# biodatageeks/polars-bio

Measured on AMD Instinct MI355X. Metric: overlap-pairs/sec, higher is better.
Workload: dtype int32; 1 GPU; overlap_100M_5M_24contig; probe_rows=100000000, build_rows=5000000, contigs=24, filter_op=Strict, parallelism=single GPU

## Files before the change

### polars-bio_amd/csrc/cslice.hip.h

```cpp
#pragma once
#include "slice.hip.h"

namespace ivj {

constexpr int CS_THREADS = 1024;
constexpr int CS_WAVES = CS_THREADS / kWave;
constexpr int CS_ITEMS = 4;
constexpr int CS_TILE = CS_THREADS * CS_ITEMS;
constexpr int CS_WTILE = kWave * CS_ITEMS;
constexpr int CS_MAX_CONTIGS = 256;
constexpr int CS_WIN = 12;
constexpr int CS_LIN = 4;
constexpr int CS_POS_BIAS = 1 << 23;
static_assert((long long)SL_MAX_BUCKETS * SL_MAX_ROWS <= CS_POS_BIAS, "an index of this path must fit a staging entry's row field");
constexpr int CS_BIN_STRIDE_PAD = 2;

constexpr int CS_CUR_STRIDE = 1;
constexpr int CS_META_FMT = 8;
constexpr unsigned long long CS_STATE_REC8 = 8ull;
constexpr int CS_REC8_GIVE_UP = 3;
__host__ __device__ __forceinline__ int cs_bits_for(uint32_t v) { int b = 0; while (b < 32 && (v >> b) != 0) ++b; return b == 0 ? 1 : b; }

typedef int cs_rec __attribute__((ext_vector_type(3), aligned(4)));
typedef int cs_rec8 __attribute__((ext_vector_type(2), aligned(8)));
// ... 687 lines not shown
    __syncthreads();
    uint32_t mlen = 0, moff = 0;
    const int64_t n_groups = (n + (int64_t)CS_SGROUP * CS_SRATE - 1) / ((int64_t)CS_SGROUP * CS_SRATE);
    for (int64_t t = (int64_t)bid * CS_THREADS + threadIdx.x; t < n_groups * CS_SGROUP; t += (int64_t)nblocks * CS_THREADS) {
        const int64_t i = (t / CS_SGROUP) * ((int64_t)CS_SGROUP * CS_SRATE) + (t % CS_SGROUP);
        if (i < n) {
            const int32_t qe = pe[i], qs = ps[i];
            const uint32_t b = cs_bucket<STRICT>(l_spl, l_cm, l_cell, g.nb, g.n_contigs, pc[i], qe);
            atomicAdd(&h[b], 1u);
            if (b < (uint32_t)g.nb) {
                const uint32_t len = qe >= qs ? (uint32_t)qe - (uint32_t)qs : 0x7fffffffu;
                const uint32_t off = (uint32_t)qe - (uint32_t)unflip((uint32_t)l_spl[b]);
                mlen = len > mlen ? len : mlen;
                moff = off > moff ? off : moff;
            }
        }
    }
#pragma unroll
    for (int d = kWave / 2; d > 0; d >>= 1) {
        const uint32_t a = __shfl_xor(mlen, d, kWave), b = __shfl_xor(moff, d, kWave);
        mlen = a > mlen ? a : mlen; moff = b > moff ? b : moff;
    }
    if ((threadIdx.x & (kWave - 1)) == 0) { atomicMax(&h[g.nb + 1], mlen); atomicMax(&h[g.nb + 2], moff); }
    __syncthreads();
    for (int k = threadIdx.x; k <= g.nb; k += CS_THREADS) if (h[k]) atomicAdd(&gh[k], h[k]);
    if (threadIdx.x == 0) { atomicMax(&gh[g.nb + 1], h[g.nb + 1]); atomicMax(&gh[g.nb + 2], h[g.nb + 2]); }
}
template <bool STRICT>
__global__ __launch_bounds__(CS_THREADS) void k_cs_sample_hist(CsTab tab, CsGeom g, const int32_t* __restrict__ pc, const int32_t* __restrict__ ps,
                                                              const int32_t* __restrict__ pe, int64_t n, uint32_t* __restrict__ gh) {
    extern __shared__ __attribute__((aligned(16))) unsigned char cs_lds[];
    cs_sample_body<STRICT>(cs_lds, blockIdx.x, gridDim.x, tab, g, pc, ps, pe, n, gh);
}
template <bool STRICT>
__global__ __launch_bounds__(CS_THREADS) void k_cs_bins_sample(int n_bins, const int32_t* __restrict__ bound, const int32_t* __restrict__ b_start,
                                                              const int2* __restrict__ ep, const int32_t* __restrict__ b_contig,
                                                              const int32_t* __restrict__ seg, int R, unsigned short* __restrict__ bins,
                                                              int4* __restrict__ smeta, int32_t* __restrict__ far_rows,
                                                              CsTab tab, CsGeom g, const int32_t* __restrict__ pc, const int32_t* __restrict__ ps,
                                                              const int32_t* __restrict__ pe, int64_t n, uint32_t* __restrict__ gh) {
    extern __shared__ __attribute__((aligned(16))) unsigned char cs_lds[];
    __shared__ uint32_t wmin[CS_WAVES];
    if ((int)blockIdx.x < n_bins) cs_bins_body(cs_lds, wmin, (int)blockIdx.x, bound, b_start, ep, b_contig, seg, R, bins, smeta, far_rows);
    else cs_sample_body<STRICT>(cs_lds, blockIdx.x - (unsigned)n_bins, gridDim.x - (unsigned)n_bins, tab, g, pc, ps, pe, n, gh);
}

__global__ __launch_bounds__(CS_THREADS) void k_cs_regions(const uint32_t* __restrict__ gh, int nb, uint32_t slack, int allow8, uint32_t* __restrict__ rstart,
                                                          uint32_t* __restrict__ rcur, int32_t* __restrict__ meta, const int32_t* __restrict__ far_src,
                                                          uint32_t* __restrict__ hw, uint32_t hw_seq) {
    if (threadIdx.x == 0 && hw) {
        hw_store(hw + 4, (uint32_t)__hip_atomic_load(far_src, __ATOMIC_RELAXED, __HIP_MEMORY_SCOPE_AGENT));
        hw_store(hw + 5, hw_seq);
    }
    if (threadIdx.x == 0) {
        int lb = 0;
        if (allow8) {
            const unsigned long long ml = (unsigned long long)gh[nb + 1] * 2ull + 64ull;
            const unsigned long long mo = (unsigned long long)gh[nb + 2] + gh[nb + 2] / 4 + 4096ull;
            const int lbits = ml > 0xffffffffull ? 33 : cs_bits_for((uint32_t)ml);
            const int obits = mo > 0xffffffffull ? 33 : cs_bits_for((uint32_t)mo);
            if (lbits + obits <= 32) lb = 32 - obits;
        }
        meta[CS_META_FMT] = lb;
    }
    __shared__ __attribute__((aligned(16))) int wsum[CS_WAVES];
    constexpr int OWN = (SL_MAX_BUCKETS + 1 + CS_THREADS - 1) / CS_THREADS;
    uint32_t cap[OWN];
    long long mine = 0;
#pragma unroll
    for (int q = 0; q < OWN; ++q) {
        const int b = OWN * threadIdx.x + q;
        cap[q] = 0;
        if (b < nb) {
            const unsigned long long est = (unsigned long long)gh[b] * CS_SRATE;
            unsigned long long c = est + est / 4 + slack;
            c = (c + 31ull) & ~31ull;
            cap[q] = (uint32_t)c;
        }
        mine += cap[q];
    }
    long long total;
    long long pre = sl_block_exclusive_sum_i32<CS_WAVES>((int)mine, wsum, &total);
#pragma unroll
    for (int q = 0; q < OWN; ++q) {
        const int b = OWN * threadIdx.x + q;
        if (b < nb) { rstart[b] = (uint32_t)pre; rcur[(size_t)b * CS_CUR_STRIDE] = 0u; }
// ... 1463 lines not shown
```

### polars-bio_amd/csrc/host_core.hip.h

```cpp
#pragma once

namespace {

thread_local std::string g_err;

int fail(int code, const std::string& msg) { g_err = msg; return code; }

#define HIP_TRY(expr)                                                                         \
    do {                                                                                      \
        hipError_t _e = (expr);                                                               \
        if (_e != hipSuccess)                                                                 \
            return fail(IVJ_EHIP, std::string(#expr) + ": " + hipGetErrorString(_e));         \
    } while (0)

#define IVJ_ABI_CATCH                                                                                     \
    catch (const std::bad_alloc&) { return fail(IVJ_ENOMEM, "host allocation failed (std::bad_alloc)"); }   \
    catch (const std::exception& e) { return fail(IVJ_ESTATE, std::string("internal error: ") + e.what()); } \
    catch (...) { return fail(IVJ_ESTATE, "internal error: unknown exception"); }

#define IVJ_TRY(expr)                 \
    do {                              \
        int _r = (expr);              \
        if (_r != IVJ_OK) return _r;  \
    } while (0)
// ... 31 lines not shown
        for (int k = 0; k < 2; ++k) {
            if (buf[k]) (void)hipHostFree(buf[k]);
            if (ev[k]) (void)hipEventDestroy(ev[k]);
            buf[k] = nullptr; ev[k] = nullptr;
        }
    }
};

inline std::atomic<int> g_live_contexts{0};

struct ivj_ctx {
    ivj_ctx() { g_live_contexts.fetch_add(1, std::memory_order_relaxed); }
    ~ivj_ctx() { g_live_contexts.fetch_sub(1, std::memory_order_relaxed); }
    ivj_ctx(const ivj_ctx&) = delete;
    ivj_ctx& operator=(const ivj_ctx&) = delete;
    int device = 0;
    hipStream_t own_stream = nullptr;
    hipStream_t stream = nullptr;
    Arena arena;
    char* ov_buf = nullptr;
    size_t ov_cap = 0;
    int64_t ov_n = -1;
    const void* ov_probe_start = nullptr;
    const void *ov_probe_contig = nullptr, *ov_probe_end = nullptr;
    const ivj_index* ov_ix = nullptr;
    int32_t ov_filter = -1;
    int32_t* ov_hi = nullptr;
    int32_t* ov_cnt = nullptr;
    long long* ov_tile = nullptr;
    long long* h_total = nullptr;
    uint32_t* hw = nullptr;
    uint32_t* hw_dev = nullptr;
    uint32_t hw_seq = 0;
    uint32_t cs_far_hw_seq = 0;
    uint32_t cs_fused_hw_seq = 0;
    int env_spin_us = 4000;
    long long hw_misses = 0;
    bool cs_prep_zero = false;
    XferSlots xfer;
    char* nl_cache = nullptr;
    size_t nl_cache_cap = 0;
    int env_nearest_lines = -1;
    char* ix_cache = nullptr;
    size_t ix_cache_cap = 0;
    int64_t ov_total = 0;
    bool ov_part = false;
    int32_t *pt_c = nullptr, *pt_s = nullptr, *pt_e = nullptr, *pt_row = nullptr;
    uint32_t* pt_off = nullptr; int pt_ntiles = 0;
    uint32_t* pt_bstart = nullptr;
    bool part_attr_set = false;
    bool os_attr_set = false;
    hipEvent_t cs_event = nullptr;
    const ivj_index* cs_far_owner = nullptr;
    hipEvent_t ix3_event = nullptr;
    bool ix3_attr_set = false;
    int env_ix_merge = -1;
    int env_ix_stage = -1;
    int env_ix_v3 = -1;
    int ix3_fallback_streak = 0;
    unsigned ix3_builds_since_fallback = 0;
    int64_t ix3_fallbacks = 0;
    struct StreamBufs { int32_t* h_in = nullptr; int32_t* d_in = nullptr; size_t in_cap = 0; char* d_out = nullptr; size_t d_out_cap = 0;
                        char* h_out = nullptr; size_t h_out_cap = 0; } st_cache[3];
    char* lb_buf = nullptr; size_t lb_cap = 0;
    char* sl_buf = nullptr;
    size_t sl_cap = 0;
    int4* sl_rec = nullptr;
    uint2* sl_cache = nullptr;
    uint32_t *sl_gh = nullptr, *sl_rstart = nullptr, *sl_rcur = nullptr, *sl_bend = nullptr;
    bool sl_sampled = false;
    uint32_t *sl_blk = nullptr, *sl_part = nullptr, *sl_bstart = nullptr;
    int32_t* sl_meta = nullptr;
    int2* sl_map = nullptr;
    long long *sl_tile = nullptr, *sl_tpart = nullptr;
    bool ov_slice = false;
    bool ov_cs = false;
    bool sl_plan_valid = false;
    int sl_items = 2;
    int env_joint_bins = 0, env_count_nolds = 0, env_count_ablate = 0;
    int sl_env_rows = 0, sl_env_chunk = 0, sl_env_notab = 0, sl_env_nobins = 0, sl_env_ablate = 0, sl_env_auto = 1, sl_env_stable = 0, sl_env_sthreads = 1024;
    SlicePlan sl_plan;
    bool cs_sattr_set = false;
    bool cs_attr_set = false;
    int cs_env_walk = -1;
    int cs_env_off = 0;
    int cs_env_ptile = 0;
    int cs_env_fill_two = 0;
    int cs_env_sampled = 1;
    int cs_env_slack = 0;
    int64_t cs_sampled_overflows = 0;
    bool cs_force_exact = false;
    int cs_env_fuse_sample = 1;
    int cs_env_rec8 = 1;
    bool cs_force_rec12 = false;
    int cs_rec8_streak = 0;
    unsigned cs_rec8_skipped = 0;
    bool cs_rec8_tried = false;
    int64_t cs_rec8_overflows = 0;
    int cs_env_nocache = 0;
    int cs_env_persist = 1;
    int cs_env_pmax = 0, cs_env_pgrain = 0;
    int cs_env_pchunks = 0;
    int n_cus = 0;
    const char* cs_env_wgtrace = nullptr;
    unsigned long long* cs_trace_buf = nullptr;
    size_t cs_trace_cap = 0;
    int timing = 0;
    bool t_open = false;
    std::vector<TimingRec> recs;
    std::vector<hipEvent_t> pool;
    size_t pool_used = 0;
    std::vector<ivj_index*> live;
    std::vector<struct ivj_stream*> streams;
    std::vector<struct ivj_comm*> comms;
};

inline void spin_relax(int i, bool crowded) {
#if !defined(__HIP_DEVICE_COMPILE__) && (defined(__x86_64__) || defined(__i386__))
    __builtin_ia32_pause();
#endif
    if (crowded && (i & 7) == 7) std::this_thread::yield();
}
template <typename Query>
inline bool spin_wait(ivj_ctx* ctx, Query&& q, hipError_t* out) {
    if (ctx->env_spin_us <= 0) return false;
// ... 36 lines not shown
    int32_t* seg = nullptr;
    int32_t* flags = nullptr;
    int32_t* e_end = nullptr;
    int32_t* e_pos = nullptr;
    int4* cmeta = nullptr;
    uint32_t* bins = nullptr;
    int4* cmeta_e = nullptr;
    uint32_t* bins_e = nullptr;
    int4* brec = nullptr;
    int4* brec_e = nullptr;
    int32_t* pargmax = nullptr;
    char* ix3_z = nullptr;
    int4* nrec = nullptr;
    int4* cmeta_j = nullptr;
    int4* crec = nullptr;
    int64_t bins_len = 0;
    bool has_end_order = false, has_end_table = false;
    bool has_argmax = false;
    int4* nline = nullptr;
    size_t nline_cap = 0;
    bool has_lines = false;
    unsigned long long* psum = nullptr;
    size_t psum_stride = 0;
    bool has_psum = false;
    bool has_flat = false;
    bool has_rec4 = false;
    unsigned long long* spl = nullptr;
    int sl_R = 0, sl_nb = 0, sl_ncells = -1;
    int4* sl_cm = nullptr;
    uint32_t* sl_cell = nullptr;
    CsGeom cs_g{0, 0, 0, 0, 0};
    bool cs_ok = false, cs_built = false;
    bool cs_far_pending = false;
    bool cs_walk = false;
    int64_t cs_far = 0;
    int32_t* cs_bound = nullptr;
    unsigned long long* cs_spl = nullptr;
    int4* cs_cm = nullptr;
    uint32_t* cs_cell = nullptr;
    unsigned short* cs_bins = nullptr;
    int4* cs_smeta = nullptr;
    int32_t* hier = nullptr;
    bool hier_built = false;
    bool tables_built = false;
    bool has_tables = true;
    char* slab = nullptr;
    size_t slab_cap = 0;
};

namespace {

struct DeviceGuard {
    int prev = -1;
    bool ok = true;
    explicit DeviceGuard(int dev) {
        if (hipGetDevice(&prev) != hipSuccess) prev = -1;
        if (prev != dev) ok = hipSetDevice(dev) == hipSuccess;
    }
    ~DeviceGuard() { if (prev >= 0) (void)hipSetDevice(prev); }
};

int arena_reserve(ivj_ctx* ctx, size_t bytes) {
    Arena& A = ctx->arena;
    A.off = 0;
    if (bytes <= A.cap) return IVJ_OK;
    HIP_TRY(hipStreamSynchronize(ctx->stream));
// ... 166 lines not shown
```

### polars-bio_amd/csrc/host_cslice.hip.h

```cpp
#pragma once

namespace {

constexpr int CS_MIN_ROWS = 3072;
bool cs_geom(int64_t n, int nc, int want_rows, CsGeom& g) {
    if (n <= 0 || nc < 1 || nc > CS_MAX_CONTIGS) return false;
    const int64_t extra = (nc < n ? nc : n) + 1;
    int64_t min_rows = CS_MIN_ROWS;
    if (const char* ev = std::getenv("IVJ_CS_MIN_ROWS")) { const int v = std::atoi(ev); if (v > 0) min_rows = v; }
    int64_t R = want_rows > 0 ? want_rows : std::max<int64_t>((n + 1023) / 1024, min_rows);
    R = (R + 63) / 64 * 64;
    if (n / R + extra > SL_MAX_BUCKETS) {
        if (extra + 8 >= SL_MAX_BUCKETS) return false;
        R = ((n + (SL_MAX_BUCKETS - extra) - 1) / (SL_MAX_BUCKETS - extra) + 63) / 64 * 64;
    }
    if (R > SL_MAX_ROWS) return false;
    g.R = (int)R;
    g.nb = (int)(n / R + extra);
    g.n_contigs = nc;
    g.cps = 0; g.ncells = 0;
    for (int cps = 4; cps >= 1 && !g.ncells; cps >>= 1) {
        const int cells = cps * g.nb + 2 * nc;
        if ((size_t)cs_part_lds(g.nb, cells, nc, 4).total <= 160 * 1024) { g.ncells = cells; g.cps = cps; }
    }
    return g.ncells != 0;
}

size_t cs_index_bytes(const CsGeom& g) {
    return align_up((size_t)(g.nb + 2) * 4) + align_up((size_t)g.nb * 8) + align_up((size_t)CS_MAX_CONTIGS * 16) + align_up((size_t)g.ncells * 4) +
           align_up((size_t)g.nb * (size_t)(2 * g.R + CS_BIN_STRIDE_PAD) * 2) + align_up((size_t)g.nb * 32);
}
void cs_index_carve(ivj_index* ix, char* p) {
    const CsGeom& g = ix->cs_g;
    ix->cs_bound = (int32_t*)p; p += align_up((size_t)(g.nb + 2) * 4);
    ix->cs_spl = (unsigned long long*)p; p += align_up((size_t)g.nb * 8);
    ix->cs_cm = (int4*)p; p += align_up((size_t)CS_MAX_CONTIGS * 16);
    ix->cs_cell = (uint32_t*)p; p += align_up((size_t)g.ncells * 4);
    ix->cs_bins = (unsigned short*)p; p += align_up((size_t)g.nb * (size_t)(2 * g.R + CS_BIN_STRIDE_PAD) * 2);
    ix->cs_smeta = (int4*)p;
}

bool cs_wanted(const ivj_ctx* ctx, const ivj_index* ix, const ivj_opts* opts) {
    if (!ix->cs_ok || ctx->cs_env_off) return false;
    if (opts->slice_rows > 0 && ((opts->slice_rows + 63) / 64 * 64) != ix->cs_g.R) return false;
    return true;
}

constexpr double CS_FAR_LIMIT = 5e-4;

struct CsSampleArgs { bool strict; const int32_t *pc, *ps, *pe; int64_t n; uint32_t* gh; unsigned sgrid; size_t lds; };

int cs_ensure_tables(ivj_ctx* ctx, ivj_index* ix, const CsSampleArgs* sample = nullptr) {
    if (ix->cs_built) return IVJ_OK;
    const CsGeom& g = ix->cs_g;
    const bool pz = ctx->cs_prep_zero && sample != nullptr;
    LAUNCH(ctx, "cs_prep", k_cs_prep, 1, CS_THREADS, (const int32_t*)ix->seg, (const int32_t*)ix->b_start, g, ix->cs_bound, ix->cs_spl, ix->cs_cm, ix->cs_cell,
           pz ? reinterpret_cast<uint32_t*>(ctx->sl_meta + 4) : (uint32_t*)nullptr, pz ? 16 : 0, pz ? ctx->sl_gh : (uint32_t*)nullptr, pz ? g.nb + 4 : 0);
    const size_t lds = (size_t)4 * g.R + (size_t)2 * (2 * g.R + 8);
    if (sample) {
        const CsTab tab{ix->cs_spl, ix->cs_cm, ix->cs_cell};
        const size_t l2 = std::max(lds, sample->lds);
        with_bool(sample->strict, [&](auto S) {
            LAUNCH_LDS(ctx, "cs_bins_sample", (k_cs_bins_sample<S>), (unsigned)g.nb + sample->sgrid, CS_THREADS, l2, g.nb, (const int32_t*)ix->cs_bound, (const int32_t*)ix->b_start,
                       (const int2*)ix->ep, (const int32_t*)ix->b_contig, (const int32_t*)ix->seg, g.R, ix->cs_bins, ix->cs_smeta, ix->flags + 1, tab, g, sample->pc, sample->ps,
                       sample->pe, sample->n, sample->gh);
        });
    } else {
        LAUNCH_LDS(ctx, "cs_bins", k_cs_bins, g.nb, CS_THREADS, lds, (const int32_t*)ix->cs_bound, (const int32_t*)ix->b_start, (const int2*)ix->ep,
                   (const int32_t*)ix->b_contig, (const int32_t*)ix->seg, g.R, ix->cs_bins, ix->cs_smeta, ix->flags + 1);
    }
    HIP_TRY(hipGetLastError());
    if (!ctx->cs_event) HIP_TRY(hipEventCreateWithFlags(&ctx->cs_event, hipEventDisableTiming));
    if (sample && ctx->hw) ctx->cs_far_hw_seq = ++ctx->hw_seq;
    else {
        ctx->cs_far_hw_seq = 0;
        HIP_TRY(hipMemcpyAsync(ctx->h_total + 5, ix->flags + 1, 4, hipMemcpyDeviceToHost, ctx->stream));
        HIP_TRY(hipEventRecord(ctx->cs_event, ctx->stream));
    }
    ix->cs_far_pending = true;
    ctx->cs_far_owner = ix;
    ix->cs_built = true;
    return IVJ_OK;
}

int cs_resolve_tables(ivj_ctx* ctx, ivj_index* ix) {
    if (!ix->cs_far_pending) return IVJ_OK;
    bool have = false;
    if (ctx->cs_far_owner == ix) {
        HIP_TRY(wait_event(ctx, ctx->cs_event));
        ctx->cs_far_owner = nullptr;
        if (ctx->cs_far_hw_seq == 0) { ix->cs_far = *reinterpret_cast<const int32_t*>(ctx->h_total + 5); have = true; }
        else if (reinterpret_cast<volatile uint32_t*>(ctx->hw)[5] == ctx->cs_far_hw_seq) { ix->cs_far = (int32_t)reinterpret_cast<volatile uint32_t*>(ctx->hw)[4]; have = true; }
        else ++ctx->hw_misses;
    }
    if (!have) {
        HIP_TRY(hipMemcpyAsync(ctx->h_total + 5, ix->flags + 1, 4, hipMemcpyDeviceToHost, ctx->stream));
        HIP_TRY(hipStreamSynchronize(ctx->stream));
        ix->cs_far = *reinterpret_cast<const int32_t*>(ctx->h_total + 5);
    }
    const double share = ix->n > 0 ? (double)ix->cs_far / (double)ix->n : 0.0;
    ix->cs_walk = ctx->cs_env_walk >= 0 ? ctx->cs_env_walk != 0 : share > CS_FAR_LIMIT;
    ix->cs_far_pending = false;
    if (ix->cs_walk) IVJ_TRY(ensure_hier(ctx, ix));
    return IVJ_OK;
}

bool cs_sampled_wanted(const ivj_ctx* ctx, int64_t n, bool stable) {
    return !stable && ctx->cs_env_sampled != 0 && !ctx->cs_force_exact && n >= (1ll << 16) && n <= (1ll << 30);
}
uint32_t cs_region_slack(const ivj_ctx* ctx, const CsGeom& g, int64_t n) {
    if (ctx->cs_env_slack > 0) return (uint32_t)((ctx->cs_env_slack + 31) & ~31);
    return (uint32_t)((4 * CS_TILE + n / (16 * (int64_t)(g.nb > 0 ? g.nb : 1)) + 31) & ~31ll);
}
int64_t cs_record_capacity(const ivj_ctx* ctx, const CsGeom& g, int64_t n) {
    return n + n / 4 + n / 32 + (int64_t)(cs_region_slack(ctx, g, n) + 64) * (g.nb + 2) + 4 * CS_TILE;
}

int cs_plan(const ivj_ctx* ctx, const ivj_index* ix, int64_t n, const ivj_opts* opts, SlicePlan& P, int& wcap) {
    const CsGeom& g = ix->cs_g;
    P.g.nb = g.nb; P.g.R = g.R; P.g.ncells = g.ncells; P.g.cps = g.cps;
    int64_t chunk = ((n + 2047) / 2048 + 2 * CS_TILE - 1) / (2 * CS_TILE) * (2 * CS_TILE);
    if (chunk < 2 * CS_TILE) chunk = 2 * CS_TILE;
    if (chunk > 16 * CS_TILE) chunk = 16 * CS_TILE;
    P.chunk = (int)chunk;
    P.nchunks = (int)((n + chunk - 1) / chunk);
    P.items = CS_ITEMS;
    const int want_chunk = opts->slice_chunk > 0 ? opts->slice_chunk : ctx->sl_env_chunk;
    int64_t jchunk = want_chunk > 0 ? ((int64_t)want_chunk + CS_TILE - 1) / CS_TILE * CS_TILE
                                    : (n >= (32ll << 20) ? 4 * CS_TILE : (n >= (8ll << 20) ? 2 * CS_TILE : CS_TILE));
    if (want_chunk <= 0 && n >= (32ll << 20)) {
        const int64_t a = n / (g.nb > 0 ? g.nb : 1);
// ... 28 lines not shown
}

int cs_partition(ivj_ctx* ctx, ivj_index* ix, const ivj_side* probe, const ivj_opts* opts, const SlicePlan& P, bool stable) {
    const int64_t n = probe->n;
    const CsGeom& g = ix->cs_g;
    const bool strict = opts->filter_op == IVJ_FILTER_STRICT;
    ctx->sl_sampled = cs_sampled_wanted(ctx, n, stable);
    const bool fuse_sample = ctx->sl_sampled && !ix->cs_built && ctx->cs_env_fuse_sample != 0;
    if (!fuse_sample) IVJ_TRY(cs_ensure_tables(ctx, ix));
    const CsTab tab{ix->cs_spl, ix->cs_cm, ix->cs_cell};
    const bool vec = aligned16(probe->contig) && aligned16(probe->start) && aligned16(probe->end) && (!probe->row_id || aligned16(probe->row_id));
    const size_t hist_lds = (size_t)16 * CS_MAX_CONTIGS + (size_t)8 * g.nb + (size_t)4 * g.ncells + 4 * (g.nb + 1);
    const size_t hist = (size_t)(g.nb + 1) * (size_t)P.nchunks;
    if (!ctx->cs_attr_set) {
        IVJ_TRY(set_dyn_lds(&k_cs_hist<true>, 96 * 1024)); IVJ_TRY(set_dyn_lds(&k_cs_hist<false>, 96 * 1024));
        IVJ_TRY(set_dyn_lds((&k_cs_scatter<true, 4, false>), 160 * 1024)); IVJ_TRY(set_dyn_lds((&k_cs_scatter<false, 4, false>), 160 * 1024));
        IVJ_TRY(set_dyn_lds((&k_cs_scatter<true, 8, false>), 160 * 1024));
        IVJ_TRY(set_dyn_lds(&k_cs_join<true, CS_FUSED>, 160 * 1024)); IVJ_TRY(set_dyn_lds(&k_cs_join<false, CS_FUSED>, 160 * 1024));
        IVJ_TRY(set_dyn_lds(&k_cs_join<true, CS_COUNT>, 160 * 1024)); IVJ_TRY(set_dyn_lds(&k_cs_join<false, CS_COUNT>, 160 * 1024));
        IVJ_TRY(set_dyn_lds(&k_cs_join<true, CS_FILL>, 160 * 1024)); IVJ_TRY(set_dyn_lds(&k_cs_join<false, CS_FILL>, 160 * 1024));
        IVJ_TRY(set_dyn_lds(&k_cs_join_plain<true, CS_FUSED>, 160 * 1024)); IVJ_TRY(set_dyn_lds(&k_cs_join_plain<false, CS_FUSED>, 160 * 1024));
        IVJ_TRY(set_dyn_lds(&k_cs_join_plain<true, CS_COUNT>, 160 * 1024)); IVJ_TRY(set_dyn_lds(&k_cs_join_plain<false, CS_COUNT>, 160 * 1024));
        IVJ_TRY(set_dyn_lds(&k_cs_join_plain<true, CS_FILL>, 160 * 1024)); IVJ_TRY(set_dyn_lds(&k_cs_join_plain<false, CS_FILL>, 160 * 1024));
        IVJ_TRY(set_dyn_lds(&k_cs_scatter_stable<true>, 160 * 1024)); IVJ_TRY(set_dyn_lds(&k_cs_scatter_stable<false>, 160 * 1024));
        IVJ_TRY(set_dyn_lds(&k_cs_fill<true, false, false>, 160 * 1024)); IVJ_TRY(set_dyn_lds(&k_cs_fill<false, false, false>, 160 * 1024));
        IVJ_TRY(set_dyn_lds(&k_cs_fill<true, false, true>, 160 * 1024)); IVJ_TRY(set_dyn_lds(&k_cs_fill<false, false, true>, 160 * 1024));
        IVJ_TRY(set_dyn_lds(&k_cs_fill<true, true, false>, 160 * 1024)); IVJ_TRY(set_dyn_lds(&k_cs_fill<false, true, false>, 160 * 1024));
        ctx->cs_attr_set = true;
    }
    int32_t* rec = reinterpret_cast<int32_t*>(ctx->sl_rec);
    if (ctx->sl_sampled) {
        if (!ctx->cs_sattr_set) {
            IVJ_TRY(set_dyn_lds(&k_cs_sample_hist<true>, 96 * 1024)); IVJ_TRY(set_dyn_lds(&k_cs_sample_hist<false>, 96 * 1024));
            IVJ_TRY(set_dyn_lds(&k_cs_bins_sample<true>, 96 * 1024)); IVJ_TRY(set_dyn_lds(&k_cs_bins_sample<false>, 96 * 1024));
            IVJ_TRY(set_dyn_lds((&k_cs_scatter<true, 4, true>), 160 * 1024)); IVJ_TRY(set_dyn_lds((&k_cs_scatter<false, 4, true>), 160 * 1024));
            IVJ_TRY(set_dyn_lds((&k_cs_scatter<true, 8, true>), 160 * 1024)); IVJ_TRY(set_dyn_lds((&k_cs_scatter<false, 8, true>), 160 * 1024));
            IVJ_TRY(set_dyn_lds((&k_cs_scatter<true, 4, true, true>), 160 * 1024)); IVJ_TRY(set_dyn_lds((&k_cs_scatter<false, 4, true, true>), 160 * 1024));
            IVJ_TRY(set_dyn_lds((&k_cs_scatter<true, 8, true, true>), 160 * 1024)); IVJ_TRY(set_dyn_lds((&k_cs_scatter<false, 8, true, true>), 160 * 1024));
            IVJ_TRY(set_dyn_lds((&k_cs_scatter12k<true, 12>), 160 * 1024)); IVJ_TRY(set_dyn_lds((&k_cs_scatter12k<false, 12>), 160 * 1024));
            IVJ_TRY(set_dyn_lds((&k_cs_scatter12k<true, 16>), 160 * 1024)); IVJ_TRY(set_dyn_lds((&k_cs_scatter12k<false, 16>), 160 * 1024));
            ctx->cs_sattr_set = true;
        }
        const bool pz = ctx->cs_prep_zero && fuse_sample;
        if (!pz) HIP_TRY(hipMemsetAsync(ctx->sl_gh, 0, (size_t)(g.nb + 4) * 4, ctx->stream));
        const int64_t n_samp = (n + CS_SRATE - 1) / CS_SRATE;
        const unsigned sgrid = (unsigned)std::min<int64_t>(256, (n_samp + CS_THREADS - 1) / CS_THREADS);
        if (fuse_sample) {
            const CsSampleArgs sa{strict, probe->contig, probe->start, probe->end, n, ctx->sl_gh, sgrid, hist_lds + 16};
            IVJ_TRY(cs_ensure_tables(ctx, ix, &sa));
        } else {
            with_bool(strict, [&](auto S) {
                LAUNCH_LDS(ctx, "cs_sample", (k_cs_sample_hist<S>), sgrid, CS_THREADS, hist_lds + 16, tab, g, probe->contig, probe->start, probe->end, n, ctx->sl_gh);
            });
        }
        const bool sticky12 = ctx->cs_rec8_streak >= CS_REC8_GIVE_UP && (++ctx->cs_rec8_skipped & 63) != 0;
        const int allow8 = (ctx->cs_env_rec8 != 0 && !ctx->cs_force_rec12 && !sticky12) ? 1 : 0;
        ctx->cs_rec8_tried = allow8 != 0;
        const bool far_hw = fuse_sample && ix->cs_far_pending && ctx->cs_far_owner == ix && ctx->cs_far_hw_seq != 0;
        LAUNCH(ctx, "cs_regions", k_cs_regions, 1, CS_THREADS, (const uint32_t*)ctx->sl_gh, g.nb, cs_region_slack(ctx, g, n), allow8, ctx->sl_rstart, ctx->sl_rcur, ctx->sl_meta,
               (const int32_t*)(ix->flags + 1), far_hw ? ctx->hw_dev : (uint32_t*)nullptr, ctx->cs_far_hw_seq);
        if (far_hw) HIP_TRY(hipEventRecord(ctx->cs_event, ctx->stream));
        unsigned long long* state = reinterpret_cast<unsigned long long*>(ctx->sl_meta + 4);
        if (allow8) t_begin(ctx, "cs_scatter");
        auto scatter = [&](auto R8) {
            with_bool(strict, P.part_items == 8, [&](auto S, auto I8) {
                hipLaunchKernelGGL((k_cs_scatter<S, I8 ? 8 : 4, true, R8>), dim3(P.nchunks), dim3(CS_THREADS), P.part_lds, ctx->stream, tab, g, probe->contig, probe->start,
                                   probe->end, probe->row_id, n, P.chunk, P.nchunks, vec, (const uint32_t*)ctx->sl_rstart, ctx->sl_rcur, state, (const int32_t*)ctx->sl_meta, rec, ctx->sl_env_ablate);
            });
        };
        if (allow8) {
            if (P.part12) {
                const int wide = (P.part16 && !probe->row_id) ? 16 : 12;
                const size_t ldsw = (size_t)cs_part12_lds(g.nb, g.ncells, g.n_contigs, wide).total;
                unsigned long long* ptrace = nullptr;
                const char* ptrace_path = std::getenv("IVJ_CS_PTRACE");
                if (ptrace_path && ptrace_path[0]) {
                    HIP_TRY(hipMalloc((void**)&ptrace, (size_t)P.nchunks * 64));
                    HIP_TRY(hipMemsetAsync(ptrace, 0, (size_t)P.nchunks * 64, ctx->stream));
                }
                with_bool(strict, wide == 16, [&](auto S, auto W16) {
                    hipLaunchKernelGGL((k_cs_scatter12k<S, W16 ? 16 : 12>), dim3(P.nchunks), dim3(CS_THREADS), ldsw, ctx->stream, tab, g, probe->contig, probe->start, probe->end, probe->row_id, n,
                                       P.chunk, P.nchunks, vec, (const uint32_t*)ctx->sl_rstart, ctx->sl_rcur, state, (const int32_t*)ctx->sl_meta, rec, ctx->sl_env_ablate, ptrace);
                });
                if (ptrace) {
                    std::vector<unsigned long long> h((size_t)P.nchunks * 8);
                    HIP_TRY(hipStreamSynchronize(ctx->stream));
                    HIP_TRY(hipMemcpy(h.data(), ptrace, h.size() * 8, hipMemcpyDeviceToHost));
                    (void)hipFree(ptrace);
                    if (FILE* f = std::fopen(ptrace_path, "ab")) {
                        const unsigned long long head[4] = {0x50545243ull, (unsigned long long)P.nchunks, (unsigned long long)P.chunk, (unsigned long long)wide};
                        std::fwrite(head, 8, 4, f); std::fwrite(h.data(), 8, h.size(), f); std::fclose(f);
                    }
                }
            }
// ... 211 lines not shown
```

### polars-bio_amd/csrc/ivjoin.hip

```cpp
#include "../../include/ivjoin.h"

#include <hip/hip_runtime.h>

#include <algorithm>
#include <atomic>
#include <chrono>
#include <cstdio>
#include <cstdlib>
#include <cstring>
#include <string>
#include <vector>
#include <thread>
#include <type_traits>

#include "probe.hip.h"
#include "slice.hip.h"
#include "cslice.hip.h"
#include "onesweep.hip.h"
#include "ixsort3.hip.h"
#include "scan.hip.h"
#include "group.hip.h"
#include "depth.hip.h"
#include "depth_sum.hip.h"
#include "depth_query.hip.h"
// ... 40 lines not shown
int ivj_ctx_create(int device, ivj_ctx** out) try {
    if (!out) return fail(IVJ_EINVAL, "out is NULL");
    int cnt = 0;
    IVJ_TRY(ivj_device_count(&cnt));
    if (device < 0 || device >= cnt) return fail(IVJ_EHIP, "no usable HIP device " + std::to_string(device) + " (device count " + std::to_string(cnt) + ")");
    HIP_TRY(hipSetDevice(device));
    ivj_ctx* ctx = new ivj_ctx();
    ctx->device = device;
    { int cus = 0; if (hipDeviceGetAttribute(&cus, hipDeviceAttributeMultiprocessorCount, device) == hipSuccess) ctx->n_cus = cus; }
    hipError_t e = hipStreamCreateWithFlags(&ctx->own_stream, hipStreamNonBlocking);
    if (e != hipSuccess) { delete ctx; return fail(IVJ_EHIP, std::string("hipStreamCreate: ") + hipGetErrorString(e)); }
    ctx->stream = ctx->own_stream;
    if (const char* ev = std::getenv("IVJ_SLICE_ITEMS")) ctx->sl_items = std::atoi(ev) == 4 ? 4 : 2;
    if (const char* ev = std::getenv("IVJ_SLICE_ROWS")) ctx->sl_env_rows = std::atoi(ev);
    if (const char* ev = std::getenv("IVJ_SLICE_CHUNK")) ctx->sl_env_chunk = std::atoi(ev);
    if (const char* ev = std::getenv("IVJ_SLICE_NOTAB")) ctx->sl_env_notab = std::atoi(ev);
    if (const char* ev = std::getenv("IVJ_SLICE_NOBINS")) ctx->sl_env_nobins = std::atoi(ev);
    if (const char* ev = std::getenv("IVJ_SLICE_ABLATE")) ctx->sl_env_ablate = std::atoi(ev);
    if (const char* ev = std::getenv("IVJ_SLICE_AUTO")) ctx->sl_env_auto = std::atoi(ev);
    if (const char* ev = std::getenv("IVJ_SLICE_STABLE")) ctx->sl_env_stable = std::atoi(ev);
    if (const char* ev = std::getenv("IVJ_SLICE_SCATTER_THREADS")) ctx->sl_env_sthreads = std::atoi(ev);
    if (const char* ev = std::getenv("IVJ_CS")) ctx->cs_env_off = std::atoi(ev) == 0 ? 1 : 0;
    if (const char* ev = std::getenv("IVJ_CS_PTILE")) ctx->cs_env_ptile = std::atoi(ev);
    if (const char* ev = std::getenv("IVJ_CS_NOCACHE")) ctx->cs_env_nocache = std::atoi(ev);
    if (const char* ev = std::getenv("IVJ_CS_PERSIST")) ctx->cs_env_persist = std::atoi(ev);
    if (const char* ev = std::getenv("IVJ_CS_PCHUNKS")) ctx->cs_env_pchunks = std::atoi(ev);
    if (const char* ev = std::getenv("IVJ_CS_PMAX")) ctx->cs_env_pmax = std::atoi(ev);
    if (const char* ev = std::getenv("IVJ_CS_PGRAIN")) ctx->cs_env_pgrain = std::atoi(ev);
    if (const char* ev = std::getenv("IVJ_CS_WGTRACE")) ctx->cs_env_wgtrace = ev[0] ? ev : nullptr;
    if (const char* ev = std::getenv("IVJ_CS_SAMPLED")) ctx->cs_env_sampled = std::atoi(ev);
    if (const char* ev = std::getenv("IVJ_CS_SLACK")) ctx->cs_env_slack = std::atoi(ev);
    if (const char* ev = std::getenv("IVJ_CS_REC8")) ctx->cs_env_rec8 = std::atoi(ev);
    if (const char* ev = std::getenv("IVJ_CS_FUSE_SAMPLE")) ctx->cs_env_fuse_sample = std::atoi(ev);
    if (const char* ev = std::getenv("IVJ_CS_FILL_TWO")) ctx->cs_env_fill_two = std::atoi(ev);
    if (const char* ev = std::getenv("IVJ_CS_WALK")) ctx->cs_env_walk = std::atoi(ev) != 0 ? 1 : 0;
    if (const char* ev = std::getenv("IVJ_JOINT_BINS")) ctx->env_joint_bins = std::atoi(ev);
    if (const char* ev = std::getenv("IVJ_COUNT_ABLATE")) ctx->env_count_ablate = std::atoi(ev);
    if (const char* ev = std::getenv("IVJ_NEAREST_LINES")) ctx->env_nearest_lines = std::atoi(ev);
    if (const char* ev = std::getenv("IVJ_COUNT_NOLDS")) ctx->env_count_nolds = std::atoi(ev);
    if (const char* ev = std::getenv("IVJ_IX_V3")) ctx->env_ix_v3 = std::atoi(ev) != 0 ? 1 : 0;
    if (const char* ev = std::getenv("IVJ_SPIN_US")) ctx->env_spin_us = std::atoi(ev);
    if (const char* ev = std::getenv("IVJ_IX_MERGE")) ctx->env_ix_merge = std::atoi(ev);
    if (const char* ev = std::getenv("IVJ_IX_STAGE")) ctx->env_ix_stage = std::atoi(ev) != 0 ? 1 : 0;
    e = hipHostMalloc((void**)&ctx->h_total, 64, hipHostMallocDefault);
    if (e != hipSuccess) { (void)hipStreamDestroy(ctx->own_stream); delete ctx; return fail(IVJ_EHIP, std::string("hipHostMalloc: ") + hipGetErrorString(e)); }
    {
        const char* ev = std::getenv("IVJ_HOST_WORDS");
        if (!(ev && std::atoi(ev) == 0)) {
            void* hp = nullptr;
            void* dp = nullptr;
            if (hipHostMalloc(&hp, 256, hipHostMallocMapped | hipHostMallocCoherent) == hipSuccess) {
                if (hipHostGetDevicePointer(&dp, hp, 0) == hipSuccess && dp) {
                    std::memset(hp, 0, 256);
                    ctx->hw = (uint32_t*)hp; ctx->hw_dev = (uint32_t*)dp;
                } else (void)hipHostFree(hp);
            }
            (void)hipGetLastError();
        }
    }
    *out = ctx;
    return IVJ_OK;
} IVJ_ABI_CATCH

namespace {
void stream_release(ivj_stream* st, bool keep_cache);
void free_stream_bufs(ivj_ctx::StreamBufs& b) {
    if (b.h_in) (void)hipHostFree(b.h_in);
    if (b.d_in) (void)hipFree(b.d_in);
    if (b.d_out) (void)hipFree(b.d_out);
    if (b.h_out) (void)hipHostFree(b.h_out);
    b = ivj_ctx::StreamBufs();
}
}

void ivj_ctx_destroy(ivj_ctx* ctx) {
    if (!ctx) return;
    DeviceGuard g(ctx->device);
    (void)hipStreamSynchronize(ctx->stream);
    while (!ctx->streams.empty()) stream_release(ctx->streams.back(), false);
    for (ivj_index* ix : ctx->live) ix->ctx = nullptr;
    for (ivj_comm* cm : ctx->comms) comm_detach(cm);
    if (ctx->arena.base) (void)hipFree(ctx->arena.base);
    if (ctx->ov_buf) (void)hipFree(ctx->ov_buf);
    if (ctx->sl_buf) (void)hipFree(ctx->sl_buf);
    if (ctx->cs_trace_buf) (void)hipFree(ctx->cs_trace_buf);
    if (ctx->lb_buf) (void)hipFree(ctx->lb_buf);
    for (auto& cb : ctx->st_cache) free_stream_bufs(cb);
    if (ctx->ix_cache) (void)hipFree(ctx->ix_cache);
    if (ctx->nl_cache) (void)hipFree(ctx->nl_cache);
    if (ctx->ix3_event) (void)hipEventDestroy(ctx->ix3_event);
    if (ctx->cs_event) (void)hipEventDestroy(ctx->cs_event);
    if (ctx->h_total) (void)hipHostFree(ctx->h_total);
    if (std::getenv("IVJ_DEBUG_REDO")) std::fprintf(stderr, "[ivj] context: host words %s, %lld misses of %u; ix3 fallbacks %lld\n", ctx->hw ? "on" : "off", (long long)ctx->hw_misses, ctx->hw_seq, (long long)ctx->ix3_fallbacks);
    if (ctx->hw) (void)hipHostFree(ctx->hw);
    ctx->xfer.release();
    for (hipEvent_t ev : ctx->pool) (void)hipEventDestroy(ev);
    if (ctx->own_stream) (void)hipStreamDestroy(ctx->own_stream);
    delete ctx;
}

int ivj_ctx_set_stream(ivj_ctx* ctx, void* hip_stream) try {
    if (!ctx) return fail(IVJ_EINVAL, "ctx is NULL");
    HIP_TRY(hipStreamSynchronize(ctx->stream));
    ctx->stream = (hip_stream == (void*)-1) ? ctx->own_stream : (hipStream_t)hip_stream;
    return IVJ_OK;
} IVJ_ABI_CATCH

int ivj_ctx_sync(ivj_ctx* ctx) try {
    if (!ctx) return fail(IVJ_EINVAL, "ctx is NULL");
    HIP_TRY(hipStreamSynchronize(ctx->stream));
    return IVJ_OK;
} IVJ_ABI_CATCH

namespace ivj { __global__ void k_profile_mark() {} }

int ivj_ctx_profile_mark(ivj_ctx* ctx) try {
    if (!ctx) return fail(IVJ_EINVAL, "ctx is NULL");
    DeviceGuard g(ctx->device);
    hipLaunchKernelGGL(ivj::k_profile_mark, dim3(1), dim3(1), 0, ctx->stream);
    HIP_TRY(hipGetLastError());
    return IVJ_OK;
} IVJ_ABI_CATCH

int ivj_ctx_enable_timing(ivj_ctx* ctx, int on) try {
// ... 10 lines not shown
    HIP_TRY(hipStreamSynchronize(ctx->stream));
    std::vector<ivj_timing> agg;
    for (const TimingRec& r : ctx->recs) {
        float ms = 0.f;
        if (hipEventElapsedTime(&ms, r.a, r.b) != hipSuccess) continue;
        size_t j = 0;
        for (; j < agg.size(); ++j) if (std::strcmp(agg[j].name, r.name) == 0) break;
        if (j == agg.size()) {
            ivj_timing t; std::memset(&t, 0, sizeof t);
            std::strncpy(t.name, r.name, sizeof(t.name) - 1);
            agg.push_back(t);
        }
        agg[j].launches += 1; agg[j].ms += ms;
    }
    *n = (int)agg.size();
    for (int i = 0; i < (int)agg.size() && i < cap; ++i) out[i] = agg[i];
    ctx->recs.clear();
    ctx->pool_used = 0;
    return IVJ_OK;
} IVJ_ABI_CATCH


int ivj_index_build_dev(ivj_ctx* ctx, const ivj_side* build_dev, const ivj_opts* opts, int with_end_order, ivj_index** out) try {
    if (!ctx || !out) return fail(IVJ_EINVAL, "ctx or out is NULL");
    IVJ_TRY(check_opts(opts));
    IVJ_TRY(check_side(build_dev, "build"));
    DeviceGuard g(ctx->device);
    return index_build(ctx, build_dev, opts, with_end_order, out);
} IVJ_ABI_CATCH

void ivj_index_free(ivj_index* ix) {
    if (!ix) return;
    ivj_ctx* ctx = ix->ctx;
    if (ctx) {
        if (ctx->ov_ix == ix) { ctx->ov_ix = nullptr; ctx->ov_n = -1; }
        for (size_t k = 0; k < ctx->live.size(); ++k)
            if (ctx->live[k] == ix) { ctx->live[k] = ctx->live.back(); ctx->live.pop_back(); break; }
    }
    if (ix->nline) {
        if (ctx && ix->nline_cap > ctx->nl_cache_cap) {
            char* old = ctx->nl_cache;
            ctx->nl_cache = reinterpret_cast<char*>(ix->nline); ctx->nl_cache_cap = ix->nline_cap;
            if (old) { DeviceGuard g(ctx->device); (void)hipFree(old); }
        } else {
            DeviceGuard g(ix->device);
            (void)hipFree(ix->nline);
        }
    }
    if (ix->psum) {
        DeviceGuard g(ix->device);
        (void)hipFree(ix->psum);
    }
    if (ix->slab) {
        if (ctx && ix->slab_cap > ctx->ix_cache_cap) {
            char* old = ctx->ix_cache;
            ctx->ix_cache = ix->slab; ctx->ix_cache_cap = ix->slab_cap;
            if (old) { DeviceGuard g(ctx->device); (void)hipFree(old); }
        } else {
            DeviceGuard g(ix->device);
            (void)hipFree(ix->slab);
        }
    }
    delete ix;
}

int ivj_overlap_count_dev(ivj_ctx* ctx, ivj_index* ix, const ivj_side* probe_dev, const ivj_opts* opts, int64_t* n_pairs) try {
// ... 1127 lines not shown
```

Measured before the change: 111.4 billion overlap-pairs/s.

## Run cs_bins on a side stream concurrently with probe sampling instead of fusing kernels

Replaces the fused bins+sample kernel with separate kernels. On first build, the bin-table kernel runs on a forked non-blocking side stream while the sampling histogram runs on the main stream. The main stream joins via an event when tables are resolved. The far-count readback moves to a pinned memcpy plus event, dropping the host-word path in the regions kernel. This adds stream, event and lifetime handling, and the benefit only applies when tables are not already built.

Result: no change. 111.8 billion overlap-pairs/s, median of 3 (+0.4%).

```diff
diff --git a/polars-bio_amd/csrc/cslice.hip.h b/polars-bio_amd/csrc/cslice.hip.h
--- a/polars-bio_amd/csrc/cslice.hip.h
+++ b/polars-bio_amd/csrc/cslice.hip.h
@@ -743,26 +743,9 @@
     extern __shared__ __attribute__((aligned(16))) unsigned char cs_lds[];
     cs_sample_body<STRICT>(cs_lds, blockIdx.x, gridDim.x, tab, g, pc, ps, pe, n, gh);
 }
-template <bool STRICT>
-__global__ __launch_bounds__(CS_THREADS) void k_cs_bins_sample(int n_bins, const int32_t* __restrict__ bound, const int32_t* __restrict__ b_start,
-                                                              const int2* __restrict__ ep, const int32_t* __restrict__ b_contig,
-                                                              const int32_t* __restrict__ seg, int R, unsigned short* __restrict__ bins,
-                                                              int4* __restrict__ smeta, int32_t* __restrict__ far_rows,
-                                                              CsTab tab, CsGeom g, const int32_t* __restrict__ pc, const int32_t* __restrict__ ps,
-                                                              const int32_t* __restrict__ pe, int64_t n, uint32_t* __restrict__ gh) {
-    extern __shared__ __attribute__((aligned(16))) unsigned char cs_lds[];
-    __shared__ uint32_t wmin[CS_WAVES];
-    if ((int)blockIdx.x < n_bins) cs_bins_body(cs_lds, wmin, (int)blockIdx.x, bound, b_start, ep, b_contig, seg, R, bins, smeta, far_rows);
-    else cs_sample_body<STRICT>(cs_lds, blockIdx.x - (unsigned)n_bins, gridDim.x - (unsigned)n_bins, tab, g, pc, ps, pe, n, gh);
-}
 
 __global__ __launch_bounds__(CS_THREADS) void k_cs_regions(const uint32_t* __restrict__ gh, int nb, uint32_t slack, int allow8, uint32_t* __restrict__ rstart,
-                                                          uint32_t* __restrict__ rcur, int32_t* __restrict__ meta, const int32_t* __restrict__ far_src,
-                                                          uint32_t* __restrict__ hw, uint32_t hw_seq) {
-    if (threadIdx.x == 0 && hw) {
-        hw_store(hw + 4, (uint32_t)__hip_atomic_load(far_src, __ATOMIC_RELAXED, __HIP_MEMORY_SCOPE_AGENT));
-        hw_store(hw + 5, hw_seq);
-    }
+                                                          uint32_t* __restrict__ rcur, int32_t* __restrict__ meta) {
     if (threadIdx.x == 0) {
         int lb = 0;
         if (allow8) {
diff --git a/polars-bio_amd/csrc/host_core.hip.h b/polars-bio_amd/csrc/host_core.hip.h
--- a/polars-bio_amd/csrc/host_core.hip.h
+++ b/polars-bio_amd/csrc/host_core.hip.h
@@ -87,7 +87,6 @@
     uint32_t* hw = nullptr;
     uint32_t* hw_dev = nullptr;
     uint32_t hw_seq = 0;
-    uint32_t cs_far_hw_seq = 0;
     uint32_t cs_fused_hw_seq = 0;
     int env_spin_us = 4000;
     long long hw_misses = 0;
@@ -107,6 +106,8 @@
     bool os_attr_set = false;
     hipEvent_t cs_event = nullptr;
     const ivj_index* cs_far_owner = nullptr;
+    hipStream_t cs_side = nullptr;
+    hipEvent_t cs_fork = nullptr;
     hipEvent_t ix3_event = nullptr;
     bool ix3_attr_set = false;
     int env_ix_merge = -1;
@@ -146,6 +147,7 @@
     int64_t cs_sampled_overflows = 0;
     bool cs_force_exact = false;
     int cs_env_fuse_sample = 1;
+    int cs_env_side = 1;
     int cs_env_rec8 = 1;
     bool cs_force_rec12 = false;
     int cs_rec8_streak = 0;
@@ -248,6 +250,7 @@
     CsGeom cs_g{0, 0, 0, 0, 0};
     bool cs_ok = false, cs_built = false;
     bool cs_far_pending = false;
+    hipEvent_t cs_side_ev = nullptr;
     bool cs_walk = false;
     int64_t cs_far = 0;
     int32_t* cs_bound = nullptr;
diff --git a/polars-bio_amd/csrc/host_cslice.hip.h b/polars-bio_amd/csrc/host_cslice.hip.h
--- a/polars-bio_amd/csrc/host_cslice.hip.h
+++ b/polars-bio_amd/csrc/host_cslice.hip.h
@@ -48,35 +48,44 @@
 
 constexpr double CS_FAR_LIMIT = 5e-4;
 
-struct CsSampleArgs { bool strict; const int32_t *pc, *ps, *pe; int64_t n; uint32_t* gh; unsigned sgrid; size_t lds; };
-
-int cs_ensure_tables(ivj_ctx* ctx, ivj_index* ix, const CsSampleArgs* sample = nullptr) {
+struct CsStreamScope {
+    ivj_ctx* ctx; hipStream_t keep;
+    CsStreamScope(ivj_ctx* c, hipStream_t s) : ctx(c), keep(c->stream) { ctx->stream = s; }
+    ~CsStreamScope() { ctx->stream = keep; }
+};
+
+int cs_ensure_tables(ivj_ctx* ctx, ivj_index* ix, bool split = false) {
     if (ix->cs_built) return IVJ_OK;
     const CsGeom& g = ix->cs_g;
-    const bool pz = ctx->cs_prep_zero && sample != nullptr;
+    const bool pz = ctx->cs_prep_zero && split;
     LAUNCH(ctx, "cs_prep", k_cs_prep, 1, CS_THREADS, (const int32_t*)ix->seg, (const int32_t*)ix->b_start, g, ix->cs_bound, ix->cs_spl, ix->cs_cm, ix->cs_cell,
            pz ? reinterpret_cast<uint32_t*>(ctx->sl_meta + 4) : (uint32_t*)nullptr, pz ? 16 : 0, pz ? ctx->sl_gh : (uint32_t*)nullptr, pz ? g.nb + 4 : 0);
-    const size_t lds = (size_t)4 * g.R + (size_t)2 * (2 * g.R + 8);
-    if (sample) {
-        const CsTab tab{ix->cs_spl, ix->cs_cm, ix->cs_cell};
-        const size_t l2 = std::max(lds, sample->lds);
-        with_bool(sample->strict, [&](auto S) {
-            LAUNCH_LDS(ctx, "cs_bins_sample", (k_cs_bins_sample<S>), (unsigned)g.nb + sample->sgrid, CS_THREADS, l2, g.nb, (const int32_t*)ix->cs_bound, (const int32_t*)ix->b_start,
-                       (const int2*)ix->ep, (const int32_t*)ix->b_contig, (const int32_t*)ix->seg, g.R, ix->cs_bins, ix->cs_smeta, ix->flags + 1, tab, g, sample->pc, sample->ps,
-                       sample->pe, sample->n, sample->gh);
-        });
-    } else {
+    HIP_TRY(hipGetLastError());
+    if (!ctx->cs_event) HIP_TRY(hipEventCreateWithFlags(&ctx->cs_event, hipEventDisableTiming));
+    hipStream_t bs = ctx->stream;
+    if (split && ctx->cs_env_side != 0) {
+        if (!ctx->cs_side) HIP_TRY(hipStreamCreateWithFlags(&ctx->cs_side, hipStreamNonBlocking));
+        if (!ctx->cs_fork) HIP_TRY(hipEventCreateWithFlags(&ctx->cs_fork, hipEventDisableTiming));
+        HIP_TRY(hipEventRecord(ctx->cs_fork, ctx->stream));
+        HIP_TRY(hipStreamWaitEvent(ctx->cs_side, ctx->cs_fork, 0));
+        bs = ctx->cs_side;
+    }
+    auto bins = [&]() -> int {
+        CsStreamScope on(ctx, bs);
+        const size_t lds = (size_t)4 * g.R + (size_t)2 * (2 * g.R + 8);
         LAUNCH_LDS(ctx, "cs_bins", k_cs_bins, g.nb, CS_THREADS, lds, (const int32_t*)ix->cs_bound, (const int32_t*)ix->b_start, (const int2*)ix->ep,
                    (const int32_t*)ix->b_contig, (const int32_t*)ix->seg, g.R, ix->cs_bins, ix->cs_smeta, ix->flags + 1);
-    }
-    HIP_TRY(hipGetLastError());
-    if (!ctx->cs_event) HIP_TRY(hipEventCreateWithFlags(&ctx->cs_event, hipEventDisableTiming));
-    if (sample && ctx->hw) ctx->cs_far_hw_seq = ++ctx->hw_seq;
-    else {
-        ctx->cs_far_hw_seq = 0;
-        HIP_TRY(hipMemcpyAsync(ctx->h_total + 5, ix->flags + 1, 4, hipMemcpyDeviceToHost, ctx->stream));
-        HIP_TRY(hipEventRecord(ctx->cs_event, ctx->stream));
-    }
+        HIP_TRY(hipGetLastError());
+        HIP_TRY(hipMemcpyAsync(ctx->h_total + 5, ix->flags + 1, 4, hipMemcpyDeviceToHost, bs));
+        HIP_TRY(hipEventRecord(ctx->cs_event, bs));
+        return IVJ_OK;
+    };
+    const int rc = bins();
+    if (rc != IVJ_OK) {
+        if (bs != ctx->stream) (void)hipStreamSynchronize(bs);
+        return rc;
+    }
+    if (bs != ctx->stream) ix->cs_side_ev = ctx->cs_event;
     ix->cs_far_pending = true;
     ctx->cs_far_owner = ix;
     ix->cs_built = true;
@@ -84,19 +93,19 @@
 }
 
 int cs_resolve_tables(ivj_ctx* ctx, ivj_index* ix) {
+    if (ix->cs_side_ev) {
+        HIP_TRY(hipStreamWaitEvent(ctx->stream, ix->cs_side_ev, 0));
+        ix->cs_side_ev = nullptr;
+    }
     if (!ix->cs_far_pending) return IVJ_OK;
-    bool have = false;
     if (ctx->cs_far_owner == ix) {
         HIP_TRY(wait_event(ctx, ctx->cs_event));
         ctx->cs_far_owner = nullptr;
-        if (ctx->cs_far_hw_seq == 0) { ix->cs_far = *reinterpret_cast<const int32_t*>(ctx->h_total + 5); have = true; }
-        else if (reinterpret_cast<volatile uint32_t*>(ctx->hw)[5] == ctx->cs_far_hw_seq) { ix->cs_far = (int32_t)reinterpret_cast<volatile uint32_t*>(ctx->hw)[4]; have = true; }
-        else ++ctx->hw_misses;
-    }
-    if (!have) {
-        HIP_TRY(hipMemcpyAsync(ctx->h_total + 5, ix->flags + 1, 4, hipMemcpyDeviceToHost, ctx->stream));
+        ix->cs_far = *reinterpret_cast<const int32_t*>(ctx->h_total + 5);
+    } else {
+        HIP_TRY(hipMemcpyAsync(ctx->h_total + 6, ix->flags + 1, 4, hipMemcpyDeviceToHost, ctx->stream));
         HIP_TRY(hipStreamSynchronize(ctx->stream));
-        ix->cs_far = *reinterpret_cast<const int32_t*>(ctx->h_total + 5);
+        ix->cs_far = *reinterpret_cast<const int32_t*>(ctx->h_total + 6);
     }
     const double share = ix->n > 0 ? (double)ix->cs_far / (double)ix->n : 0.0;
     ix->cs_walk = ctx->cs_env_walk >= 0 ? ctx->cs_env_walk != 0 : share > CS_FAR_LIMIT;
@@ -191,7 +200,6 @@
     if (ctx->sl_sampled) {
         if (!ctx->cs_sattr_set) {
             IVJ_TRY(set_dyn_lds(&k_cs_sample_hist<true>, 96 * 1024)); IVJ_TRY(set_dyn_lds(&k_cs_sample_hist<false>, 96 * 1024));
-            IVJ_TRY(set_dyn_lds(&k_cs_bins_sample<true>, 96 * 1024)); IVJ_TRY(set_dyn_lds(&k_cs_bins_sample<false>, 96 * 1024));
             IVJ_TRY(set_dyn_lds((&k_cs_scatter<true, 4, true>), 160 * 1024)); IVJ_TRY(set_dyn_lds((&k_cs_scatter<false, 4, true>), 160 * 1024));
             IVJ_TRY(set_dyn_lds((&k_cs_scatter<true, 8, true>), 160 * 1024)); IVJ_TRY(set_dyn_lds((&k_cs_scatter<false, 8, true>), 160 * 1024));
             IVJ_TRY(set_dyn_lds((&k_cs_scatter<true, 4, true, true>), 160 * 1024)); IVJ_TRY(set_dyn_lds((&k_cs_scatter<false, 4, true, true>), 160 * 1024));
@@ -204,21 +212,14 @@
         if (!pz) HIP_TRY(hipMemsetAsync(ctx->sl_gh, 0, (size_t)(g.nb + 4) * 4, ctx->stream));
         const int64_t n_samp = (n + CS_SRATE - 1) / CS_SRATE;
         const unsigned sgrid = (unsigned)std::min<int64_t>(256, (n_samp + CS_THREADS - 1) / CS_THREADS);
-        if (fuse_sample) {
-            const CsSampleArgs sa{strict, probe->contig, probe->start, probe->end, n, ctx->sl_gh, sgrid, hist_lds + 16};
-            IVJ_TRY(cs_ensure_tables(ctx, ix, &sa));
-        } else {
-            with_bool(strict, [&](auto S) {
-                LAUNCH_LDS(ctx, "cs_sample", (k_cs_sample_hist<S>), sgrid, CS_THREADS, hist_lds + 16, tab, g, probe->contig, probe->start, probe->end, n, ctx->sl_gh);
-            });
-        }
+        if (fuse_sample) IVJ_TRY(cs_ensure_tables(ctx, ix, true));
+        with_bool(strict, [&](auto S) {
+            LAUNCH_LDS(ctx, "cs_sample", (k_cs_sample_hist<S>), sgrid, CS_THREADS, hist_lds + 16, tab, g, probe->contig, probe->start, probe->end, n, ctx->sl_gh);
+        });
         const bool sticky12 = ctx->cs_rec8_streak >= CS_REC8_GIVE_UP && (++ctx->cs_rec8_skipped & 63) != 0;
         const int allow8 = (ctx->cs_env_rec8 != 0 && !ctx->cs_force_rec12 && !sticky12) ? 1 : 0;
         ctx->cs_rec8_tried = allow8 != 0;
-        const bool far_hw = fuse_sample && ix->cs_far_pending && ctx->cs_far_owner == ix && ctx->cs_far_hw_seq != 0;
-        LAUNCH(ctx, "cs_regions", k_cs_regions, 1, CS_THREADS, (const uint32_t*)ctx->sl_gh, g.nb, cs_region_slack(ctx, g, n), allow8, ctx->sl_rstart, ctx->sl_rcur, ctx->sl_meta,
-               (const int32_t*)(ix->flags + 1), far_hw ? ctx->hw_dev : (uint32_t*)nullptr, ctx->cs_far_hw_seq);
-        if (far_hw) HIP_TRY(hipEventRecord(ctx->cs_event, ctx->stream));
+        LAUNCH(ctx, "cs_regions", k_cs_regions, 1, CS_THREADS, (const uint32_t*)ctx->sl_gh, g.nb, cs_region_slack(ctx, g, n), allow8, ctx->sl_rstart, ctx->sl_rcur, ctx->sl_meta);
         unsigned long long* state = reinterpret_cast<unsigned long long*>(ctx->sl_meta + 4);
         if (allow8) t_begin(ctx, "cs_scatter");
         auto scatter = [&](auto R8) {
diff --git a/polars-bio_amd/csrc/ivjoin.hip b/polars-bio_amd/csrc/ivjoin.hip
--- a/polars-bio_amd/csrc/ivjoin.hip
+++ b/polars-bio_amd/csrc/ivjoin.hip
@@ -96,6 +96,7 @@
     if (const char* ev = std::getenv("IVJ_CS_SLACK")) ctx->cs_env_slack = std::atoi(ev);
     if (const char* ev = std::getenv("IVJ_CS_REC8")) ctx->cs_env_rec8 = std::atoi(ev);
     if (const char* ev = std::getenv("IVJ_CS_FUSE_SAMPLE")) ctx->cs_env_fuse_sample = std::atoi(ev);
+    if (const char* ev = std::getenv("IVJ_CS_SIDE")) ctx->cs_env_side = std::atoi(ev);
     if (const char* ev = std::getenv("IVJ_CS_FILL_TWO")) ctx->cs_env_fill_two = std::atoi(ev);
     if (const char* ev = std::getenv("IVJ_CS_WALK")) ctx->cs_env_walk = std::atoi(ev) != 0 ? 1 : 0;
     if (const char* ev = std::getenv("IVJ_JOINT_BINS")) ctx->env_joint_bins = std::atoi(ev);
@@ -141,8 +142,9 @@
     if (!ctx) return;
     DeviceGuard g(ctx->device);
     (void)hipStreamSynchronize(ctx->stream);
+    if (ctx->cs_side) (void)hipStreamSynchronize(ctx->cs_side);
     while (!ctx->streams.empty()) stream_release(ctx->streams.back(), false);
-    for (ivj_index* ix : ctx->live) ix->ctx = nullptr;
+    for (ivj_index* ix : ctx->live) { ix->ctx = nullptr; ix->cs_side_ev = nullptr; }
     for (ivj_comm* cm : ctx->comms) comm_detach(cm);
     if (ctx->arena.base) (void)hipFree(ctx->arena.base);
     if (ctx->ov_buf) (void)hipFree(ctx->ov_buf);
@@ -154,6 +156,8 @@
     if (ctx->nl_cache) (void)hipFree(ctx->nl_cache);
     if (ctx->ix3_event) (void)hipEventDestroy(ctx->ix3_event);
     if (ctx->cs_event) (void)hipEventDestroy(ctx->cs_event);
+    if (ctx->cs_fork) (void)hipEventDestroy(ctx->cs_fork);
+    if (ctx->cs_side) (void)hipStreamDestroy(ctx->cs_side);
     if (ctx->h_total) (void)hipHostFree(ctx->h_total);
     if (std::getenv("IVJ_DEBUG_REDO")) std::fprintf(stderr, "[ivj] context: host words %s, %lld misses of %u; ix3 fallbacks %lld\n", ctx->hw ? "on" : "off", (long long)ctx->hw_misses, ctx->hw_seq, (long long)ctx->ix3_fallbacks);
     if (ctx->hw) (void)hipHostFree(ctx->hw);
@@ -230,6 +234,11 @@
 void ivj_index_free(ivj_index* ix) {
     if (!ix) return;
     ivj_ctx* ctx = ix->ctx;
+    if (ix->cs_side_ev) {
+        DeviceGuard g(ix->device);
+        (void)hipEventSynchronize(ix->cs_side_ev);
+        ix->cs_side_ev = nullptr;
+    }
     if (ctx) {
         if (ctx->ov_ix == ix) { ctx->ov_ix = nullptr; ctx->ov_n = -1; }
         for (size_t k = 0; k < ctx->live.size(); ++k)
```
